# OPPOMKLab/u-LLaVA

Hardware: AMD Instinct MI355X
Metric: images/sec/GPU (ViT-L-336 + LLaMA-7B + SAM RES forward) at 1/2/4/8 MI355X (higher is better)
Workload: dtype bf16; 1 GPU; C4: ViT-L/14-336 + LLaMA-7B instruct forward, 336x336 image + 64-token prompt (S=643), batch 32/GPU; per_gpu_batch=32, global_batch=32, seq_len=643, image=336, parallelism=dp1, weights=random-init N(0,0.02), ViT-L/14 + LLaMA-7B (V=32011) shapes

## Files before the change

### u-llava_amd/csrc/attention.hip

```cpp
#include "ull_common.h"
#include <stdlib.h>
#include <type_traits>

#include "attention_common.h"

namespace {

typedef uint32_t u32x2_t __attribute__((ext_vector_type(2)));
template <int OFF>
ULL_DEV u32x2_t lds_tr_b64(uint32_t addr) {
    u32x2_t v;
    asm volatile("ds_read_b64_tr_b16 %0, %1 offset:%2" : "=v"(v) : "v"(addr), "n"(OFF) : "memory");
    return v;
}
template <int N, int LEFT = 0>
ULL_DEV void lds_tr_wait(u32x2_t (&a)[N], u32x2_t (&b)[N]) {
    static_assert(N == 1 || N == 4 || N == 5 || N == 8, "head-dim blocks of hd = 64 / 80 / 128");
    if constexpr (N == 1)
        asm volatile("s_waitcnt lgkmcnt(%2)" : "+v"(a[0]), "+v"(b[0]) : "n"(LEFT) : "memory");
    else if constexpr (N == 4)
        asm volatile("s_waitcnt lgkmcnt(%8)" : "+v"(a[0]), "+v"(a[1]), "+v"(a[2]), "+v"(a[3]), "+v"(b[0]), "+v"(b[1]), "+v"(b[2]), "+v"(b[3])
                     : "n"(LEFT) : "memory");
    else if constexpr (N == 5)
        asm volatile("s_waitcnt lgkmcnt(%10)"
                     : "+v"(a[0]), "+v"(a[1]), "+v"(a[2]), "+v"(a[3]), "+v"(a[4]), "+v"(b[0]), "+v"(b[1]), "+v"(b[2]), "+v"(b[3]), "+v"(b[4])
                     : "n"(LEFT) : "memory");
    else
        asm volatile("s_waitcnt lgkmcnt(%16)"
                     : "+v"(a[0]), "+v"(a[1]), "+v"(a[2]), "+v"(a[3]), "+v"(a[4]), "+v"(a[5]), "+v"(a[6]), "+v"(a[7]), "+v"(b[0]), "+v"(b[1]),
                       "+v"(b[2]), "+v"(b[3]), "+v"(b[4]), "+v"(b[5]), "+v"(b[6]), "+v"(b[7])
                     : "n"(LEFT) : "memory");
}

template <int HDP, int NT, int NWV, bool EXACT, bool VROW>
constexpr int attn_reg_nbuf() {
    constexpr int ULL_ATTN_RING = 2;
    return EXACT ? 2 * NT : ((VROW && (HDP / 8) % NWV == 0 && NT >= 2) ? ULL_ATTN_RING : 2);
}

template <int HDP, int NT, int FL, int NWV, bool EXACT = false, bool VROW = false>
__global__ __launch_bounds__(NWV * 64, (EXACT || (VROW && HDP == 64 && NWV == 4)) ? 4 : (VROW && HDP == 128 && NT <= 11 && NWV <= 4) ? 3 :
                                       2)
void attn_reg_kernel(AttnArgs p) {
    extern __shared__ __attribute__((aligned(256))) char smem[];
    static_assert(!VROW || ((FL == FL_LLAMA || FL == FL_CLIP) && HDP >= 64), "VROW: flavors that pin hd = HDP");
    constexpr int PM = HDP / 16 >= 8 ? 7 : HDP / 16 - 1;
    constexpr int BQ = 16 * NWV;
    constexpr int CPR = HDP / 8;
    constexpr int KROW = HDP * 2;
    constexpr int NKS = HDP / 32, NDS = HDP / 16;
    constexpr int TILE = 64 * KROW > HDP * 128 ? 64 * KROW : HDP * 128;
    const int tid = threadIdx.x, lane = tid & 63;
    const int hd = head_dim_of<HDP, FL>(p);
    const int wave = __builtin_amdgcn_readfirstlane(tid >> 6);
    const int fr = lane & 15, fg = lane >> 4;

    const int nq = (p.Sq + BQ - 1) / BQ;
    const int xcd = blockIdx.x & 7, slot = blockIdx.x >> 3;
    const int head = (slot / nq) * 8 + xcd;
    if (head >= p.B * p.H) return;
    const int qt = nq - 1 - slot % nq;
    const int b = head / p.H, h = head % p.H;
    const int q0 = qt * BQ;
    const int koff = p.Sk - p.Sq;

    const uint32_t lds_base = __builtin_amdgcn_readfirstlane((uint32_t)(uintptr_t)(__attribute__((address_space(3))) char*)smem);
    constexpr int NBUF = attn_reg_nbuf<HDP, NT, NWV, EXACT, VROW>();
    constexpr int PPW = (CPR + NWV - 1) / NWV;
    char* maskb = smem + NBUF * TILE;
    elem_t* biasb = (elem_t*)(smem + NBUF * TILE + NT * KT);

    int kend = p.Sk;
    if (p.causal) kend = min(p.Sk, q0 + BQ + koff);
    if (kend < 1) kend = 1;
    const int nkt = EXACT ? NT : (kend + KT - 1) / KT;
    int kend_w = p.Sk;
    if (p.causal) kend_w = min(p.Sk, q0 + wave * 16 + 16 + koff);
    int nkt_w = EXACT ? NT : (q0 + wave * 16 < p.Sq) ? max(1, (kend_w + KT - 1) / KT) : 0;

    const elem_t* kbase = p.K + (long)b * p.k_bs + (long)h * p.k_hs;
    const elem_t* vbase = p.Vt + (long)b * p.vt_bs + (long)h * p.vt_hs;
    constexpr bool FASTDMA = VROW && (HDP / 8) % NWV == 0;
    uint32_t kvo[FASTDMA ? 2 * PPW : 1];
    if constexpr (FASTDMA) {
#pragma unroll
        for (int i0 = 0; i0 < PPW; ++i0) {
            const int i = i0 * NWV + wave;
            const int row = i * (64 / CPR) + lane / CPR;
            const int ck = (lane % CPR) ^ swz<CPR>(row);
            const int cpos = lane % CPR;
            const int cv = ((((cpos >> 1) ^ (row & PM)) << 1) | (cpos & 1));
            kvo[i0] = (uint32_t)(((long)row * p.k_ss + ck * 8) * 2);
            kvo[PPW + i0] = (uint32_t)(((long)row * p.vt_ds + cv * 8) * 2);
        }
    }
    const bool fast_dma_ok = FASTDMA && 64 * p.k_ss * 2 < (1L << 31) && 64 * p.vt_ds * 2 < (1L << 31);
    auto issue = [&](int s) {
        const uint32_t dst = lds_base + (EXACT ? s : (s % NBUF)) * TILE;
        if constexpr (FASTDMA) {
            const int kt = s < nkt ? s : s - nkt;
            if (fast_dma_ok && kt * KT + KT <= p.Sk) {
                const elem_t* tb = s < nkt ? kbase + (long)kt * KT * p.k_ss : vbase + (long)kt * KT * p.vt_ds;
#pragma unroll
                for (int i0 = 0; i0 < PPW; ++i0) glds16s(tb, s < nkt ? kvo[i0] : kvo[PPW + i0], dst + (i0 * NWV + wave) * 1024);
                return;
            }
        }
        if (s < nkt) {
            const int kt = s;
#pragma unroll
            for (int i0 = 0; i0 < CPR; i0 += NWV) {
                const int i = i0 + wave;
                if (i < CPR) {
                    const int row = i * (64 / CPR) + lane / CPR;
                    const int c = (lane % CPR) ^ swz<CPR>(row);
                    const int key = min(kt * KT + row, p.Sk - 1);
                    const elem_t* krow = kbase + (long)key * p.k_ss;
                    const elem_t* src = (c * 8 < hd) ? krow + c * 8 : p.zeros;
                    glds16(src, dst + i * 1024);
                }
            }
        } else if constexpr (VROW) {
            const int kt = s - nkt;
#pragma unroll
            for (int i0 = 0; i0 < CPR; i0 += NWV) {
                const int i = i0 + wave;
                if (i < CPR) {
                    const int row = i * (64 / CPR) + lane / CPR;
                    const int cpos = lane % CPR;
                    const int c = ((((cpos >> 1) ^ (row & PM)) << 1) | (cpos & 1));
                    const int key = min(kt * KT + row, p.Sk - 1);
                    glds16(vbase + (long)key * p.vt_ds + c * 8, dst + i * 1024);
                }
            }
        } else {
            const int kt = s - nkt;
            const int npieces = hd >> 3;
#pragma unroll
            for (int i0 = 0; i0 < HDP / 8; i0 += NWV) {
                const int i = i0 + wave;
                if (i < npieces) {
                    const int row = i * 8 + (lane >> 3);
                    const int c = (lane & 7) ^ (row & 7);
                    glds16(vbase + (long)row * p.vt_ds + kt * KT + c * 8, dst + i * 1024);
                }
            }
        }
    };

    if constexpr (EXACT) {
#pragma unroll
        for (int kt = 0; kt < NT; ++kt) issue(kt);
    } else {
#pragma unroll
        for (int s0 = 0; s0 < NBUF - 1; ++s0)
            if (s0 < 2 * nkt) issue(s0);
    }

    uint4 qf[NKS];
    const int qi = q0 + wave * 16 + fr;
    {
        const elem_t* qp = p.Q + (long)b * p.q_bs + (long)h * p.q_hs + (long)qi * p.q_ss;
#pragma unroll
        for (int ks = 0; ks < NKS; ++ks) {
            const int d = ks * 32 + fg * 8;
            qf[ks] = (qi < p.Sq && d < hd) ? *(const uint4*)(qp + d) : make_uint4(0, 0, 0, 0);
        }
        for (int j = tid; j < nkt * KT; j += NWV * 64) {
            unsigned char m = 2;
            if (j < p.Sk) m = (p.key_mask == nullptr || p.key_mask[(long)b * p.Sk + j] != 0) ? 1 : 0;
            maskb[j] = m;
        }
    }
    const elem_t* brow = nullptr;
    int bh_off = 0, bw_off = 0;
    if (p.rel_h != nullptr) {
        const int bp = bias_pitch(p);
        stage_rel_bias<NKS>(p, biasb + wave * 16 * bp, bp, qf, q0 + wave * 16, head, lane, bh_off, bw_off, hd);
        brow = biasb + (wave * 16 + fr) * bp;
    }
    if (p.q_scale != 1.0f) {
#pragma unroll
        for (int ks = 0; ks < NKS; ++ks) qf[ks] = scale_q8(qf[ks], p.q_scale);
    }
    asm volatile("s_waitcnt vmcnt(0)" ::: "memory");
#pragma unroll
    for (int ks = 0; ks < NKS; ++ks) asm volatile("" : "+v"(qf[ks].x), "+v"(qf[ks].y), "+v"(qf[ks].z), "+v"(qf[ks].w));
    float mrow = -INFINITY;
    ULL_ATT_ACC(0, stamp_t);

    uint32_t sp[NT][8];
    uint32_t kfo[NKS];
#pragma unroll
    for (int ks = 0; ks < NKS; ++ks) {
        kfo[ks] = fr * KROW + (((ks * 4 + fg) ^ swz<CPR>(fr)) << 4);
        asm volatile("" : "+v"(kfo[ks]));
    }
    uint32_t vfo = (4 * fg + (fr >> 2)) * KROW + ((fr & 2) << 3) + ((fr & 1) << 3) + (((4 * (fg & 1) + (fr >> 2)) & PM) << 5);
    asm volatile("" : "+v"(vfo));
    if constexpr (EXACT) {
        __builtin_amdgcn_s_barrier();
#pragma unroll
        for (int kt = 0; kt < NT; ++kt) issue(NT + kt);
    }
    auto stream_step = [&](int s) {
        const int total = 2 * nkt;
        const int later = min(NBUF - 2, total - 1 - s);
        if (NBUF >= 4 && later >= 2) asm volatile("s_waitcnt vmcnt(%0)" :: "n"(2 * PPW) : "memory");
        else if (NBUF >= 3 && later == 1) asm volatile("s_waitcnt vmcnt(%0)" :: "n"(PPW) : "memory");
        else asm volatile("s_waitcnt vmcnt(0)" ::: "memory");
        __builtin_amdgcn_s_barrier();
        if (s + NBUF - 1 < total) issue(s + NBUF - 1);
    };

#pragma clang loop unroll(full)
    for (int kt = 0; kt < NT; ++kt) {
        if (kt < nkt) {
            if constexpr (!EXACT) stream_step(kt);
            ULL_ATT_ACC(1, stamp_t);
            if (kt < nkt_w) {
                const char* tb = smem + (EXACT ? kt : (kt % NBUF)) * TILE;
                if constexpr (VROW) {
                    if (p.key_mask == nullptr && kt * KT + KT <= p.Sk && (FL != FL_LLAMA || kt * KT + KT - 1 <= q0 + wave * 16 + koff)) {
constexpr int ULL_ATTN_CHAINS = 2;
#pragma unroll
                        for (int n0 = 0; n0 < 4; n0 += ULL_ATTN_CHAINS) {
                            f32x4_t accn[ULL_ATTN_CHAINS];
#pragma unroll
                            for (int c = 0; c < ULL_ATTN_CHAINS; ++c) accn[c] = f32x4_t{0.f, 0.f, 0.f, 0.f};
#pragma unroll
                            for (int ks = 0; ks < NKS; ++ks)
#pragma unroll
                                for (int c = 0; c < ULL_ATTN_CHAINS; ++c) {
                                    const uint4 kf = *(const uint4*)(tb + (n0 + c) * 16 * KROW + kfo[ks]);
                                    accn[c] = mfma16(kf, qf[ks], accn[c]);
                                }
#pragma unroll
                            for (int c = 0; c < ULL_ATTN_CHAINS; ++c)
                                score_quad_clean<FL>(p, accn[c], sp[kt][(n0 + c) * 2], sp[kt][(n0 + c) * 2 + 1], &mrow);
                        }
                        continue;
                    }
                }
#pragma unroll
                for (int ns = 0; ns < 4; ++ns) {
                    f32x4_t acc = {0.f, 0.f, 0.f, 0.f};
                    const int row = ns * 16 + fr;
#pragma unroll
                    for (int ks = 0; ks < NKS; ++ks) {
                        if (ks * 32 < hd) {
                            const uint4 kf = *(const uint4*)(tb + ns * 16 * KROW + kfo[ks]);
                            acc = mfma16(kf, qf[ks], acc);
                        }
                    }
                    if constexpr (FL == FL_LLAMA || FL == FL_CLIP) {
                        if (p.key_mask == nullptr && kt * KT + KT <= p.Sk && (FL != FL_LLAMA || kt * KT + KT - 1 <= q0 + wave * 16 + koff)) {
                            score_quad_clean<FL>(p, acc, sp[kt][ns * 2], sp[kt][ns * 2 + 1], &mrow);
                            continue;
                        }
                    }
                    const uint32_t mk = *(const uint32_t*)(maskb + kt * KT + ns * 16 + fg * 4);
                    const int j0 = kt * KT + ns * 16 + fg * 4;
                    bool fast = false;
                    if constexpr (FL == FL_LLAMA || FL == FL_CLIP) {
                        const bool dirty = mk != 0x01010101u || (FL == FL_LLAMA && j0 + 3 > qi + koff);
                        fast = __builtin_amdgcn_ballot_w64(dirty) == 0;
                    }
                    if (fast) score_quad_clean<FL>(p, acc, sp[kt][ns * 2], sp[kt][ns * 2 + 1], &mrow);
                    else score_quad<FL>(p, acc, j0, mk, qi, koff, brow, bh_off, bw_off, sp[kt][ns * 2], sp[kt][ns * 2 + 1], &mrow);
                    if constexpr (EXACT) __builtin_amdgcn_sched_barrier(0);
                }
            }
        }
    }

    {
        float m = rnd(mrow);
        m = fmaxf(m, __shfl_xor(m, 16, 64));
        m = fmaxf(m, __shfl_xor(m, 32, 64));
        float sum = 0.f;
#pragma clang loop unroll(full)
        for (int kt = 0; kt < NT; ++kt)
            if (kt < nkt_w) {
#pragma unroll
                for (int i = 0; i < 8; ++i) {
                    const f32x2_t t = (f32x2_t{pk_lo(sp[kt][i]), pk_hi(sp[kt][i])} - m) * 1.4426950408889634f;
                    sum += __builtin_amdgcn_exp2f(t.x);
                    sum += __builtin_amdgcn_exp2f(t.y);
                }
                if constexpr (EXACT) __builtin_amdgcn_sched_barrier(0);
            }
        sum += __shfl_xor(sum, 16, 64);
        sum += __shfl_xor(sum, 32, 64);
        const float inv = 1.0f / sum;
#pragma clang loop unroll(full)
        for (int kt = 0; kt < NT; ++kt)
            if (kt < nkt_w) {
#pragma unroll
                for (int i = 0; i < 8; ++i) {
                    const f32x2_t t = (f32x2_t{pk_lo(sp[kt][i]), pk_hi(sp[kt][i])} - m) * 1.4426950408889634f;
                    const f32x2_t e = f32x2_t{__builtin_amdgcn_exp2f(t.x), __builtin_amdgcn_exp2f(t.y)} * inv;
                    sp[kt][i] = pack2e(e.x, e.y);
                }
                if constexpr (EXACT) __builtin_amdgcn_sched_barrier(0);
            }
    }

    f32x4_t oacc[NDS];
#pragma unroll
    for (int ds = 0; ds < NDS; ++ds) oacc[ds] = f32x4_t{0.f, 0.f, 0.f, 0.f};
    if constexpr (EXACT) {
        asm volatile("s_waitcnt vmcnt(0)" ::: "memory");
        __builtin_amdgcn_s_barrier();
    }
#pragma clang loop unroll(full)
    for (int kt = 0; kt < NT; ++kt) {
        if (kt < nkt) {
            if constexpr (!EXACT) stream_step(nkt + kt);
            ULL_ATT_ACC(4, stamp_t);
            if constexpr (VROW) {
                if (kt < nkt_w) {
                    const uint32_t vb = lds_base + (EXACT ? NT + kt : ((nkt + kt) % NBUF)) * TILE + vfo;
#pragma unroll
                    for (int kk = 0; kk < 2; ++kk) {
                        const uint4 pf = make_uint4(sp[kt][4 * kk], sp[kt][4 * kk + 1], sp[kt][4 * kk + 2], sp[kt][4 * kk + 3]);
#pragma unroll
                        for (int d0 = 0; d0 < NDS; d0 += 4) {
                            u32x2_t va[4], vc[4];
#pragma unroll
                            for (int j = 0; j < 4; ++j) {
                                const uint32_t ad = vb ^ ((d0 + j) << 5);
                                if (kk == 0) { va[j] = lds_tr_b64<0>(ad); vc[j] = lds_tr_b64<16 * KROW>(ad); }
                                else { va[j] = lds_tr_b64<32 * KROW>(ad); vc[j] = lds_tr_b64<48 * KROW>(ad); }
                            }
                            lds_tr_wait<4>(va, vc);
#pragma unroll
                            for (int j = 0; j < 4; ++j)
                                oacc[d0 + j] = mfma16(make_uint4(va[j].x, va[j].y, vc[j].x, vc[j].y), pf, oacc[d0 + j]);
                        }
                    }
                }
            } else
            if (kt < nkt_w) {
                const char* tb = smem + (EXACT ? NT + kt : ((nkt + kt) % NBUF)) * TILE;
#pragma unroll
                for (int kk = 0; kk < 2; ++kk) {
                    const uint4 pf = make_uint4(sp[kt][4 * kk], sp[kt][4 * kk + 1], sp[kt][4 * kk + 2], sp[kt][4 * kk + 3]);
#pragma unroll
                    for (int ds = 0; ds < NDS; ++ds) {
                        if (ds * 16 < hd) {
                            const int row = ds * 16 + fr;
                            const uint4 vf = *(const uint4*)(tb + row * 128 + (((kk * 4 + fg) ^ (row & 7)) << 4));
                            oacc[ds] = mfma16(vf, pf, oacc[ds]);
                        }
                    }
                    if constexpr (EXACT) __builtin_amdgcn_sched_barrier(0);
                }
            }
        }
    }
    if constexpr (VROW && !EXACT && NBUF == 2 && NWV * 16 * KROW <= TILE) {
        char* ob = smem + ((2 * nkt - 2) % NBUF) * TILE + wave * 16 * KROW;
        constexpr int SM = CPR >= 16 ? 15 : CPR - 1;
        int ln = lane;
        asm volatile("" : "+v"(ln));
        const int er = ln & 15, eg = ln >> 4;
#pragma unroll
        for (int ds = 0; ds < NDS; ++ds) {
            uint2 pk;
            pk.x = pack2e(oacc[ds][0], oacc[ds][1]);
            pk.y = pack2e(oacc[ds][2], oacc[ds][3]);
            *(uint2*)(ob + er * KROW + ((((ds * 2 + (eg >> 1)) ^ (er & SM))) << 4) + ((eg & 1) << 3)) = pk;
        }
        constexpr int RPI = 64 / CPR;
        elem_t* ow = p.O + (long)b * p.o_bs + (long)h * p.o_hs;
#pragma unroll
        for (int it = 0; it < 16 / RPI; ++it) {
            const int r = it * RPI + ln / CPR, c = ln % CPR;
            const uint4 v = *(const uint4*)(ob + r * KROW + ((c ^ (r & SM)) << 4));
            const int q = q0 + wave * 16 + r;
            if (q < p.Sq) *(uint4*)(ow + (long)q * p.o_ss + c * 8) = v;
        }
    } else
    if (qi < p.Sq) {
        elem_t* op = p.O + (long)b * p.o_bs + (long)h * p.o_hs + (long)qi * p.o_ss;
#pragma unroll
        for (int ds = 0; ds < NDS; ++ds) {
            if (ds * 16 < hd) {
                uint2 pk;
                pk.x = pack2e(oacc[ds][0], oacc[ds][1]);
                pk.y = pack2e(oacc[ds][2], oacc[ds][3]);
                *(uint2*)(op + ds * 16 + fg * 4) = pk;
            }
        }
    }
}

constexpr int SW_NWV = 13, SW_NT = 4, SW_WS = 14, SW_HD = 80, SW_NTAB = 2 * SW_WS - 1, SW_BW = SW_NTAB + 1, SW_BP = 2 * SW_BW, SW_TILE = 64 * 256;
constexpr int SW_LDS = 2 * SW_NT * SW_TILE + SW_NWV * 16 * SW_BP * 2 + 2 * SW_NTAB * SW_HD * 2;
static_assert(SW_LDS <= 160 * 1024, "K + V tiles, 208 bias rows and the two rel-pos tables fit one CU's LDS");
__global__ __launch_bounds__(SW_NWV * 64) void sam_window_kernel(AttnArgs p, int n_items) {
    extern __shared__ __attribute__((aligned(256))) char smem[];
    constexpr int NWV = SW_NWV, NT = SW_NT, WS = SW_WS, NBLK = SW_WS, KROW = 256, TILE = SW_TILE, NKS = 3, HD = SW_HD, NTAB = SW_NTAB, BW = SW_BW, BP = SW_BP;
    const int tid = threadIdx.x, lane = tid & 63;
    const int wave = __builtin_amdgcn_readfirstlane(tid >> 6);
    const int fr = lane & 15, fg = lane >> 4;
    const uint32_t lds_base = __builtin_amdgcn_readfirstlane((uint32_t)(uintptr_t)(__attribute__((address_space(3))) char*)smem);
    elem_t* biasb = (elem_t*)(smem + 2 * NT * TILE);
    elem_t* tabs = biasb + NWV * 16 * BP;
    elem_t* brow = biasb + (wave * 16 + fr) * BP;

    int item = (int)((uint64_t)blockIdx.x * (uint64_t)n_items / gridDim.x);
    const int last = (int)((uint64_t)(blockIdx.x + 1) * (uint64_t)n_items / gridDim.x);
    if (item >= last) return;

    const int qi = wave * 16 + fr;
    const int qy = min(qi, WS * WS - 1) / WS;
    const elem_t* brow_h = biasb + (wave * 16 + fr) * BP + qy + WS - 1;
    uint32_t kfo[NKS];
#pragma unroll
    for (int ks = 0; ks < NKS; ++ks) {
        kfo[ks] = fr * KROW + (((ks * 4 + fg) ^ (fr & 15)) << 4);
        asm volatile("" : "+v"(kfo[ks]));
    }
    uint32_t vfx = (lds_base + NT * TILE + (4 * fg + (fr >> 2)) * 256 + ((fr & 2) << 3) + ((fr & 1) << 3)) ^ ((4 * (fg & 1) + (fr >> 2)) << 5);
    asm volatile("" : "+v"(vfx));
    const uint32_t row_pitch = (uint32_t)p.img_w * (uint32_t)p.k_ss * 2u;

    struct Item { int h, iy0, ix0; long tok0; };
    auto locate = [&](int it) {
        const int b = udiv_magic(it, p.mg_h);
        const WinOrigin wo = win_origin(p, b, WS);
        return Item{it - b * p.H, wo.iy0, wo.ix0, ((long)wo.img * p.img_h + wo.iy0) * p.img_w + wo.ix0};
    };
    auto issue_tiles = [&](const Item& t, int which) {
        int ln = tid;
        asm volatile("" : "+v"(ln));
        const char* in_base = (const char*)((which ? p.Vt : p.K) + t.tok0 * p.k_ss + (long)t.h * p.k_hs);
        const char* pad_base = (const char*)((which ? p.v_pad : p.k_pad) + (long)t.h * p.k_hs);
#pragma unroll
        for (int j = 0; j < 2; ++j) {
            const int i = wave + j * NWV;
            if (i < 16) {
                const int l4 = (ln >> 4) & 3, cpos = ln & 15, row = i * 4 + l4;
                const uint32_t c = 16u * (uint32_t)(which ? ((((cpos >> 1) ^ (row & 7)) << 1) | (cpos & 1)) : (cpos ^ (row & 15)));
                const int lx = min((i & 3) * 4 + l4, WS - 1);
                const bool real = c < HD * 2;
                const bool col_ok = real && t.ix0 + lx < p.img_w;
                const char* in = in_base + ((uint32_t)lx * (uint32_t)p.k_ss * 2u + c);
                const char* out = real ? pad_base + c : (const char*)p.zeros;
#pragma unroll
                for (int kt = 0; kt < NT; ++kt) {
                    if (kt * 64 + i * 4 >= NBLK * 16) continue;
                    const int ly = kt * 4 + (i >> 2);
                    const bool row_ok = t.iy0 + ly < p.img_h;
                    glds16((row_ok && col_ok) ? in + (uint32_t)ly * row_pitch : out, lds_base + (which * NT + kt) * TILE + i * 1024);
                }
            }
        }
    };
    auto query_pos = [&](const Item& t, int pitch, uint32_t& off, bool& ok) {
        int ln = tid;
        asm volatile("" : "+v"(ln));
        const int q = (ln >> 6) * 16 + (ln & 15), qc = min(q, WS * WS - 1), y = qc / WS, x = qc - y * WS;
        ok = q < WS * WS && t.iy0 + y < p.img_h && t.ix0 + x < p.img_w;
        off = (uint32_t)(y * p.img_w + x) * (uint32_t)pitch * 2u;
    };
    auto load_q = [&](const Item& t, uint4 (&q)[NKS], bool& ok) {
        uint32_t off;
        query_pos(t, (int)p.q_ss, off, ok);
        int ln = tid;
        asm volatile("" : "+v"(ln));
        const int g = (ln >> 4) & 3;
        const char* qb = (const char*)(p.Q + t.tok0 * p.q_ss + (long)t.h * p.q_hs) + (off + g * 16);
#pragma unroll
        for (int ks = 0; ks < NKS; ++ks)
            q[ks] = (ok && ks * 32 + g * 8 < HD) ? *(const uint4*)(qb + ks * 64) : make_uint4(0, 0, 0, 0);
// ... 1319 lines not shown
                sp[t][i] = pack2e(lo, hi);
            }
#pragma unroll
            for (int kk = 0; kk < 2; ++kk) {
                const uint4 pf = make_uint4(sp[t][4 * kk], sp[t][4 * kk + 1], sp[t][4 * kk + 2], sp[t][4 * kk + 3]);
#pragma unroll
                for (int ds = 0; ds < NDS; ++ds) {
                    if (ds * 16 < hd) {
                        uint4 vf;
                        if constexpr (TPW == 1) vf = vpre[kk][ds];
                        else vf = *(const uint4*)(vbase + (long)(ds * 16 + fr) * p.vt_ds + kt * KT + (kk * 4 + fg) * 8);
                        oacc[ds] = mfma16(vf, pf, oacc[ds]);
                    }
                }
            }
        }
    }
#pragma unroll
    for (int ds = 0; ds < NDS; ++ds)
#pragma unroll
        for (int r = 0; r < 4; ++r) obuf[(wave * NDS * 4 + ds * 4 + r) * 64 + lane] = oacc[ds][r];
    __syncthreads();
    for (int e = tid; e < NDS * 4 * 64; e += blockDim.x) {
        float acc = 0.f;
        for (int w = 0; w < nwv; ++w) acc += obuf[w * NDS * 4 * 64 + e];
        const int reg = e >> 6, ln = e & 63;
        const int q = ln & 15, d = (reg >> 2) * 16 + (ln >> 4) * 4 + (reg & 3);
        if (q < p.Sq && d < hd) p.O[(long)b * p.o_bs + (long)h * p.o_hs + (long)q * p.o_ss + d] = f2e(acc);
    }
}

__global__ __launch_bounds__(256) void rope_inplace_kernel(elem_t* __restrict__ x, long row_stride, const int64_t* __restrict__ pos,
                                                           const float* __restrict__ inv_freq, int n_heads, int hd, float sin_sign) {
    const long tok = blockIdx.x;
    const int half = hd >> 1;
    const int cpr = half >> 3;
    const int c = threadIdx.x % cpr;
    const float pf = (float)pos[tok];
    float cs[8], sn[8];
#pragma unroll
    for (int j = 0; j < 8; ++j) {
        const float a = pf * inv_freq[c * 8 + j];
        cs[j] = rnd(cosf(a));
        sn[j] = rnd(sinf(a)) * sin_sign;
    }
    elem_t* xr = x + tok * row_stride;
    for (int hh = threadIdx.x / cpr; hh < n_heads; hh += blockDim.x / cpr) {
        elem_t* p1 = xr + hh * hd + c * 8;
        elem_t* p2 = p1 + half;
        float a[8], bb[8], o1[8], o2[8];
        unpack8(*(const uint4*)p1, a);
        unpack8(*(const uint4*)p2, bb);
#pragma unroll
        for (int j = 0; j < 8; ++j) {
            o1[j] = rnd(a[j] * cs[j]) + rnd(-bb[j] * sn[j]);
            o2[j] = rnd(bb[j] * cs[j]) + rnd(a[j] * sn[j]);
        }
        *(uint4*)p1 = pack8(o1);
        *(uint4*)p2 = pack8(o2);
    }
}

__global__ __launch_bounds__(256) void rope_table_kernel(const int64_t* __restrict__ pos, const float* __restrict__ inv_freq, long tokens,
                                                         int half, elem_t* __restrict__ cs, elem_t* __restrict__ sn) {
    const long total = tokens * half;
    for (long i = (long)blockIdx.x * 256 + threadIdx.x; i < total; i += (long)gridDim.x * 256) {
        const float a = (float)pos[i / half] * inv_freq[i % half];
        cs[i] = f2e(cosf(a));
        sn[i] = f2e(sinf(a));
    }
}

__global__ __launch_bounds__(64) void rope_append_kernel(elem_t* __restrict__ qkv, long row_stride, const int64_t* __restrict__ pos,
                                                         const float* __restrict__ inv_freq, int S, int H, int hd, elem_t* __restrict__ kc,
                                                         elem_t* __restrict__ vtc, int smax, int past) {
    const long tok = blockIdx.x;
    const int h = blockIdx.y;
    const int b = (int)(tok / S), s = (int)(tok % S);
    const int half = hd >> 1;
    const int cpr = half >> 3;
    elem_t* xr = qkv + tok * row_stride;
    const int slot_k = past + s;
    if ((int)threadIdx.x < 2 * cpr) {
        const int c = threadIdx.x % cpr;
        const bool is_k = (int)threadIdx.x >= cpr;
        const float pf = (float)pos[tok];
        float cs[8], sn[8];
#pragma unroll
        for (int j = 0; j < 8; ++j) {
            const float a = pf * inv_freq[c * 8 + j];
            cs[j] = rnd(cosf(a));
            sn[j] = rnd(sinf(a));
        }
        elem_t* p1 = xr + ((is_k ? H : 0) + h) * hd + c * 8;
        elem_t* p2 = p1 + half;
        float a[8], bb[8], o1[8], o2[8];
        unpack8(*(const uint4*)p1, a);
        unpack8(*(const uint4*)p2, bb);
#pragma unroll
        for (int j = 0; j < 8; ++j) {
            o1[j] = rnd(a[j] * cs[j]) + rnd(-bb[j] * sn[j]);
            o2[j] = rnd(bb[j] * cs[j]) + rnd(a[j] * sn[j]);
        }
        const uint4 r1 = pack8(o1), r2 = pack8(o2);
        if (!is_k) {
            *(uint4*)p1 = r1;
            *(uint4*)p2 = r2;
        } else {
            elem_t* kp = kc + (((long)b * H + h) * smax + slot_k) * hd + c * 8;
            *(uint4*)kp = r1;
            *(uint4*)(kp + half) = r2;
        }
    }
    const int w = slot_k & 31;
    const int slot_v = (slot_k & ~31) + 8 * ((w >> 2) & 3) + 4 * (w >> 4) + (w & 3);
    const elem_t* vr = xr + 2 * H * hd + h * hd;
    for (int i = threadIdx.x; i < hd; i += 64) vtc[(((long)b * H + h) * hd + i) * smax + slot_v] = vr[i];
}

__global__ __launch_bounds__(256) void transpose_v_kernel(const elem_t* __restrict__ v, long v_bs, long v_ss, elem_t* __restrict__ vt, int S,
                                                          int H, int hd, int pitch) {
    __shared__ __attribute__((aligned(16))) elem_t t[64][68];
    const int b = blockIdx.z / H, h = blockIdx.z % H;
    const int s0 = blockIdx.x * 64, d0 = blockIdx.y * 64;
    const elem_t* vp = v + (long)b * v_bs + (long)h * hd;
#pragma unroll
    for (int k = 0; k < 2; ++k) {
        const int c = threadIdx.x + 256 * k;
        const int sl = c >> 3, dc = (c & 7) * 8;
        uint4 val = make_uint4(0, 0, 0, 0);
        if (s0 + sl < S && d0 + dc < hd) val = *(const uint4*)(vp + (long)(s0 + sl) * v_ss + d0 + dc);
        const uint32_t w[4] = {val.x, val.y, val.z, val.w};
#pragma unroll
        for (int j = 0; j < 4; ++j) {
            t[dc + 2 * j][sl] = (elem_t)(w[j] & 0xffff);
            t[dc + 2 * j + 1][sl] = (elem_t)(w[j] >> 16);
        }
    }
    __syncthreads();
    elem_t* op = vt + ((long)b * H + h) * hd * pitch;
#pragma unroll
    for (int k = 0; k < 2; ++k) {
        const int c = threadIdx.x + 256 * k;
        const int d = c >> 3, oc = c & 7;
        const int kb = (oc >> 2) * 32 + (oc & 3) * 4;
        const uint2 lo = *(const uint2*)&t[d][kb], hi = *(const uint2*)&t[d][kb + 16];
        if (d0 + d < hd) *(uint4*)(op + (long)(d0 + d) * pitch + s0 + oc * 8) = make_uint4(lo.x, lo.y, hi.x, hi.y);
    }
}

template <int HDP, int NT, int FL, int NWV = 8, bool EXACT = false, bool VROW = false>
int launch_attn(const AttnArgs& a, hipStream_t st) {
    constexpr int TILE = 64 * HDP * 2 > HDP * 128 ? 64 * HDP * 2 : HDP * 128;
    const int lds = attn_reg_nbuf<HDP, NT, NWV, EXACT, VROW>() * TILE + NT * KT +
                    (a.rel_h ? NWV * 16 * (((a.rel_mode == 2 ? 2 * (a.KH + a.KW) - 2 : a.KH + a.KW) | 1)) * 2 + 16 : 0);
    if (lds > 160 * 1024) return ULL_ERR_LDS;
    static UllOncePerDevice once;
    if (lds > 64 * 1024 && once.first())
        (void)hipFuncSetAttribute((const void*)attn_reg_kernel<HDP, NT, FL, NWV, EXACT, VROW>, hipFuncAttributeMaxDynamicSharedMemorySize, 160 * 1024);
    const int nq = (a.Sq + 16 * NWV - 1) / (16 * NWV);
    const int nheads = a.B * a.H;
    const dim3 grid(((nheads + 7) / 8) * 8 * nq);
    hipLaunchKernelGGL((attn_reg_kernel<HDP, NT, FL, NWV, EXACT, VROW>), grid, dim3(NWV * 64), lds, st, a);
    return ull_check_launch();
}

template <int HDP, int FL>
int launch_long(const AttnArgs& a, hipStream_t st) {
    constexpr int TILE = 64 * HDP * 2;
    const int nt = (a.Sk + KT - 1) / KT;
    const int lds = 4 * TILE + ((nt * KT + 15) & ~15) + (a.rel_h ? 8 * 16 * (((a.rel_mode == 2 ? 2 * (a.KH + a.KW) - 2 : a.KH + a.KW) | 1)) * 2 + 16 : 0);
    if (lds > 160 * 1024) return ULL_ERR_LDS;
    static UllOncePerDevice once;
    if (once.first()) (void)hipFuncSetAttribute((const void*)attn_long_kernel<HDP, FL>, hipFuncAttributeMaxDynamicSharedMemorySize, 160 * 1024);
    const int nq = (a.Sq + 127) / 128;
    const dim3 grid(((a.B * a.H + 7) / 8) * 8 * nq);
    hipLaunchKernelGGL((attn_long_kernel<HDP, FL>), grid, dim3(512), lds, st, a);
    return ull_check_launch();
}

template <int HDP, int FL, int HOIST, bool VROW = false>
int launch_stream(const AttnArgs& a, hipStream_t st) {
    constexpr int TILE = 64 * HDP * 2;
    static_assert(!VROW || HOIST == 2, "row-major V: the SAM global-attention form");
    const int nt = (a.Sk + KT - 1) / KT;
    int lds = 4 * TILE;
    if (HOIST == 0) lds += ((nt * KT + 15) & ~15) + (a.rel_h ? 8 * 16 * (((a.rel_mode == 2 ? 2 * (a.KH + a.KW) - 2 : a.KH + a.KW) | 1)) * 2 + 16 : 0);
    if (lds > 160 * 1024) return ULL_ERR_LDS;
    static UllOncePerDevice once;
    if (once.first()) (void)hipFuncSetAttribute((const void*)attn_stream_kernel<HDP, FL, HOIST, VROW>, hipFuncAttributeMaxDynamicSharedMemorySize, 160 * 1024);
    const int nq = (a.Sq + 127) / 128;
    const dim3 grid(((a.B * a.H + 7) / 8) * 8 * nq);
    hipLaunchKernelGGL((attn_stream_kernel<HDP, FL, HOIST, VROW>), grid, dim3(512), lds, st, a);
    return ull_check_launch();
}

int launch_sam_global(const AttnArgs& a, hipStream_t st) {
    constexpr int LDS = 4 * 64 * 256 + 4 * 32 * 64 * 2;
    static UllOncePerDevice once;
    if (once.first()) (void)hipFuncSetAttribute((const void*)sam_global_kernel, hipFuncAttributeMaxDynamicSharedMemorySize, 160 * 1024);
    const int nq = a.Sq / 128;
    const dim3 grid(((a.B * a.H + 7) / 8) * 8 * nq);
    hipLaunchKernelGGL(sam_global_kernel, grid, dim3(256), LDS, st, a);
    return ull_check_launch();
}

int launch_sam_global_exact(const AttnArgs& a, hipStream_t st) {
    constexpr int LDS = 4 * 64 * 256 + 4 * 32 * 64 * 2;
    static UllOncePerDevice once;
    if (once.first()) (void)hipFuncSetAttribute((const void*)sam_global_exact_kernel, hipFuncAttributeMaxDynamicSharedMemorySize, 160 * 1024);
    const int nq = a.Sq / 128;
    const dim3 grid(((a.B * a.H + 7) / 8) * 8 * nq);
    hipLaunchKernelGGL(sam_global_exact_kernel, grid, dim3(256), LDS, st, a);
    return ull_check_launch();
}

template <int HDP, int FL, int TPW>
int launch_fewq_t(const AttnArgs& a, int nwv, hipStream_t st) {
    const int lds = 2 * 16 * 16 * 4 + nwv * HDP * 16 * 4;
    static UllOncePerDevice once;
    if (once.first()) (void)hipFuncSetAttribute((const void*)attn_fewq_kernel<HDP, FL, TPW>, hipFuncAttributeMaxDynamicSharedMemorySize, 160 * 1024);
    hipLaunchKernelGGL((attn_fewq_kernel<HDP, FL, TPW>), dim3(a.B * a.H), dim3(nwv * 64), lds, st, a);
    return ull_check_launch();
}

template <int HDP, int FL>
int launch_fewq(const AttnArgs& a, hipStream_t st) {
    const int nt = (a.Sk + KT - 1) / KT;
    const int nwv = nt < 16 ? nt : 16;
    return nt <= 16 ? launch_fewq_t<HDP, FL, 1>(a, nwv, st) : launch_fewq_t<HDP, FL, 4>(a, nwv, st);
}

int flavor_of(const AttnArgs& a) {
    if (a.scale_mode == 1 && a.causal && !a.rel_h && a.q_scale == 1.0f) return FL_LLAMA;
    if (a.scale_mode == 1 && !a.causal && !a.rel_h && !a.key_mask && a.q_scale == 1.0f) return FL_CLIP;
    if (a.scale_mode == 0 && !a.causal && a.rel_h && !a.key_mask) return FL_SAM_ENC;
    if (a.scale_mode == 2 && !a.causal && !a.rel_h && !a.key_mask && a.q_scale == 1.0f) return FL_SAM_DEC;
    return FL_RUNTIME;
}

template <int HDP>
int dispatch_nt(const AttnArgs& a, hipStream_t st) {
    const int nt = (a.Sk + KT - 1) / KT;
    int fl = flavor_of(a);
    if ((fl == FL_LLAMA || fl == FL_CLIP) && a.hd != HDP) fl = FL_RUNTIME;
    if (fl == FL_SAM_ENC && HDP == 128 && a.hd != 80) fl = FL_RUNTIME;
    if (a.v_rows) {
        if constexpr (HDP == 128) {
            constexpr int ULL_ATTN_NWV = 4;
            if (fl == FL_LLAMA && a.Sq > 16 && nt <= 11) return launch_attn<128, 11, FL_LLAMA, ULL_ATTN_NWV, false, true>(a, st);
            if (fl == FL_LLAMA && a.Sq > 16 && nt <= 16) return launch_attn<128, 16, FL_LLAMA, 8, false, true>(a, st);
            if (fl == FL_SAM_ENC && a.rel_mode == 2 && a.KW == 64 && a.KH == 64 && a.Sk == 4096 && (a.Sq & 15) == 0 && a.Sq > 16 &&
                64 * a.k_ss * 2 < (1L << 31) && 64 * a.vt_ds * 2 < (1L << 31)) {
                if ((a.Sq & 127) == 0 && a.Sq == a.Sk && a.hd == 80 && !a.key_mask && !a.causal) return launch_sam_global(a, st);
                return launch_stream<128, FL_SAM_ENC, 2, true>(a, st);
            }
        }
        if constexpr (HDP == 64) {
            if (fl == FL_CLIP && a.Sq > 16 && nt <= 5) return launch_attn<64, 5, FL_CLIP, 8, false, true>(a, st);
            if (fl == FL_CLIP && a.Sq > 16 && nt <= 11) return launch_attn<64, 11, FL_CLIP, 4, false, true>(a, st);
        }
        return ULL_ERR_SHAPE;
    }
    if (a.Sq <= 16 && !a.rel_h && nt >= 2 && nt <= 64) {
        if constexpr (HDP == 128) {
            if (fl == FL_LLAMA) return launch_fewq<HDP, FL_LLAMA>(a, st);
        }
        if constexpr (HDP == 32) {
            if (fl == FL_SAM_DEC) return launch_fewq<HDP, FL_SAM_DEC>(a, st);
        }
        return launch_fewq<HDP, FL_RUNTIME>(a, st);
    }
    if constexpr (HDP == 128) {
        if (fl == FL_LLAMA && nt <= 11) return launch_attn<128, 11, FL_LLAMA, 4>(a, st);
        if (fl == FL_LLAMA && nt <= 16) return launch_attn<128, 16, FL_LLAMA>(a, st);
        if (a.win16) {
            if (fl != FL_SAM_ENC || a.KH != 14 || a.KW != 14 || a.Sk != 196 || a.Sq != 196 || a.key_mask) return ULL_ERR_SHAPE;
            const int n_items = a.B * a.H, n_cu = ull_cu_count();
            static UllOncePerDevice once;
            if (once.first()) (void)hipFuncSetAttribute((const void*)sam_window_kernel, hipFuncAttributeMaxDynamicSharedMemorySize, 160 * 1024);
            hipLaunchKernelGGL(sam_window_kernel, dim3(n_items < n_cu ? n_items : n_cu), dim3(SW_NWV * 64), SW_LDS, st, a, n_items);
            return ull_check_launch();
        }
        if (fl == FL_SAM_ENC && nt == 4 && a.Sq <= 208) return launch_attn<128, 4, FL_SAM_ENC, 13, true>(a, st);
        if (fl == FL_SAM_ENC && nt <= 11) return launch_attn<128, 11, FL_SAM_ENC>(a, st);
        if (fl == FL_SAM_ENC && nt > 16) {
            if (a.rel_mode == 1 && a.KW == KT && (a.Sk % KT) == 0) return launch_stream<128, FL_SAM_ENC, 1>(a, st);
            if (a.rel_mode == 2 && a.KW == 64 && a.KH == 64 && a.Sk == 4096 && (a.Sq & 15) == 0) return launch_stream<128, FL_SAM_ENC, 2>(a, st);
            return launch_stream<128, FL_SAM_ENC, 0>(a, st);
        }
    }
    if constexpr (HDP == 64) {
        if (fl == FL_CLIP && nt <= 5) return launch_attn<64, 5, FL_CLIP>(a, st);
        if (fl == FL_CLIP && nt <= 11) return launch_attn<64, 11, FL_CLIP, 4>(a, st);
    }
    if constexpr (HDP == 32) {
        if (fl == FL_SAM_DEC && nt <= 5) return launch_attn<32, 5, FL_SAM_DEC>(a, st);
        if (fl == FL_SAM_DEC && nt > 16) return launch_long<32, FL_SAM_DEC>(a, st);
    }
    if constexpr (HDP < 128) {
        if (nt <= 5) return launch_attn<HDP, 5, FL_RUNTIME>(a, st);
    }
    if (nt <= 11) return launch_attn<HDP, 11, FL_RUNTIME>(a, st);
    if (nt <= 16) return launch_attn<HDP, 16, FL_RUNTIME>(a, st);
    return launch_long<HDP, FL_RUNTIME>(a, st);
}

// ... 143 lines not shown
```

Before: 143.6 images/sec (whole job, all GPUs).

## Skip masked causal key groups and detect all-ones key masks in attention

Each block now checks at load time whether the key mask holds any zeros, and shares that flag through LDS so an all-ones mask can take the unmasked fast score path. For causal and CLIP variants, it also skips the QK MFMAs, the exp work and half of the PV MFMAs for 16-key groups that lie entirely past the wave's causal limit. Those groups get constant fill scores. The skip is only used when the row max is far enough above the fill value that skipped entries would contribute nothing. The cost is extra branches, a ballot and a barrier-dependent LDS read, plus 16 more bytes of LDS.

```diff
diff --git a/u-llava_amd/csrc/attention.hip b/u-llava_amd/csrc/attention.hip
--- a/u-llava_amd/csrc/attention.hip
+++ b/u-llava_amd/csrc/attention.hip
@@ -77,6 +77,11 @@
     int kend_w = p.Sk;
     if (p.causal) kend_w = min(p.Sk, q0 + wave * 16 + 16 + koff);
     int nkt_w = EXACT ? NT : (q0 + wave * 16 < p.Sq) ? max(1, (kend_w + KT - 1) / KT) : 0;
+    constexpr bool GROUPS = VROW && !EXACT && (FL == FL_LLAMA || FL == FL_CLIP);
+    const int ng_w = nkt_w > 0 ? max(1, (kend_w + 15) >> 4) : 0;
+    constexpr bool MFLAG = FL == FL_LLAMA && !EXACT;
+    char* cleanb = smem + NBUF * TILE + NT * KT;
+    bool mclean = p.key_mask == nullptr;
 
     const elem_t* kbase = p.K + (long)b * p.k_bs + (long)h * p.k_hs;
     const elem_t* vbase = p.Vt + (long)b * p.vt_bs + (long)h * p.vt_hs;
@@ -166,10 +171,28 @@
             const int d = ks * 32 + fg * 8;
             qf[ks] = (qi < p.Sq && d < hd) ? *(const uint4*)(qp + d) : make_uint4(0, 0, 0, 0);
         }
-        for (int j = tid; j < nkt * KT; j += NWV * 64) {
-            unsigned char m = 2;
-            if (j < p.Sk) m = (p.key_mask == nullptr || p.key_mask[(long)b * p.Sk + j] != 0) ? 1 : 0;
-            maskb[j] = m;
+        constexpr int MI = (NT * KT + NWV * 64 - 1) / (NWV * 64);
+        int mw[MI];
+#pragma unroll
+        for (int it = 0; it < MI; ++it) {
+            const int j = tid + it * NWV * 64;
+            mw[it] = (p.key_mask != nullptr && j < nkt * KT && j < p.Sk) ? p.key_mask[(long)b * p.Sk + j] : 1;
+        }
+        bool mzero = false;
+#pragma unroll
+        for (int it = 0; it < MI; ++it) {
+            const int j = tid + it * NWV * 64;
+            if (j < nkt * KT) {
+                const unsigned char m = j < p.Sk ? (mw[it] != 0 ? 1 : 0) : 2;
+                maskb[j] = m;
+                mzero |= m == 0;
+            }
+        }
+        if constexpr (MFLAG) {
+            if (p.key_mask != nullptr) {
+                const bool wclean = __builtin_amdgcn_ballot_w64(mzero) == 0;
+                if (lane == 0) cleanb[wave] = wclean ? 1 : 0;
+            }
         }
     }
     const elem_t* brow = nullptr;
@@ -218,10 +241,18 @@
         if (kt < nkt) {
             if constexpr (!EXACT) stream_step(kt);
             ULL_ATT_ACC(1, stamp_t);
+            if constexpr (MFLAG) {
+                if (kt == 0 && p.key_mask != nullptr) {
+                    bool c = true;
+#pragma unroll
+                    for (int w = 0; w < NWV; ++w) c &= cleanb[w] != 0;
+                    mclean = __builtin_amdgcn_readfirstlane(c) != 0;
+                }
+            }
             if (kt < nkt_w) {
                 const char* tb = smem + (EXACT ? kt : (kt % NBUF)) * TILE;
                 if constexpr (VROW) {
-                    if (p.key_mask == nullptr && kt * KT + KT <= p.Sk && (FL != FL_LLAMA || kt * KT + KT - 1 <= q0 + wave * 16 + koff)) {
+                    if (mclean && kt * KT + KT <= p.Sk && (FL != FL_LLAMA || kt * KT + KT - 1 <= q0 + wave * 16 + koff)) {
 constexpr int ULL_ATTN_CHAINS = 2;
 #pragma unroll
                         for (int n0 = 0; n0 < 4; n0 += ULL_ATTN_CHAINS) {
@@ -244,6 +275,18 @@
                 }
 #pragma unroll
                 for (int ns = 0; ns < 4; ++ns) {
+                    if constexpr (GROUPS) {
+                        if (kt * 4 + ns >= ng_w) {
+                            const int j0 = kt * KT + ns * 16 + fg * 4;
+                            float o[4];
+#pragma unroll
+                            for (int r = 0; r < 4; ++r) o[r] = j0 + r < p.Sk ? ELEM_MIN_F : -INFINITY;
+                            mrow = fmaxf(mrow, o[0]);
+                            sp[kt][ns * 2] = pack2e(o[0], o[1]);
+                            sp[kt][ns * 2 + 1] = pack2e(o[2], o[3]);
+                            continue;
+                        }
+                    }
                     f32x4_t acc = {0.f, 0.f, 0.f, 0.f};
                     const int row = ns * 16 + fr;
 #pragma unroll
@@ -254,7 +297,7 @@
                         }
                     }
                     if constexpr (FL == FL_LLAMA || FL == FL_CLIP) {
-                        if (p.key_mask == nullptr && kt * KT + KT <= p.Sk && (FL != FL_LLAMA || kt * KT + KT - 1 <= q0 + wave * 16 + koff)) {
+                        if (mclean && kt * KT + KT <= p.Sk && (FL != FL_LLAMA || kt * KT + KT - 1 <= q0 + wave * 16 + koff)) {
                             score_quad_clean<FL>(p, acc, sp[kt][ns * 2], sp[kt][ns * 2 + 1], &mrow);
                             continue;
                         }
@@ -274,19 +317,35 @@
         }
     }
 
+    int ng_phase3 = 0;
     {
         float m = rnd(mrow);
         m = fmaxf(m, __shfl_xor(m, 16, 64));
         m = fmaxf(m, __shfl_xor(m, 32, 64));
+        int ng_p = ng_w;
+        if constexpr (GROUPS) {
+            const bool far = m - ELEM_MIN_F > 256.0f && m < INFINITY;
+            if (__builtin_amdgcn_ballot_w64(!far) != 0) ng_p = nkt_w * 4;
+        }
         float sum = 0.f;
 #pragma clang loop unroll(full)
         for (int kt = 0; kt < NT; ++kt)
             if (kt < nkt_w) {
-#pragma unroll
-                for (int i = 0; i < 8; ++i) {
-                    const f32x2_t t = (f32x2_t{pk_lo(sp[kt][i]), pk_hi(sp[kt][i])} - m) * 1.4426950408889634f;
-                    sum += __builtin_amdgcn_exp2f(t.x);
-                    sum += __builtin_amdgcn_exp2f(t.y);
+                if (!GROUPS || kt * 4 + 4 <= ng_p) {
+#pragma unroll
+                    for (int i = 0; i < 8; ++i) {
+                        const f32x2_t t = (f32x2_t{pk_lo(sp[kt][i]), pk_hi(sp[kt][i])} - m) * 1.4426950408889634f;
+                        sum += __builtin_amdgcn_exp2f(t.x);
+                        sum += __builtin_amdgcn_exp2f(t.y);
+                    }
+                } else {
+#pragma unroll
+                    for (int i = 0; i < 8; ++i)
+                        if (kt * 4 + i / 2 < ng_p) {
+                            const f32x2_t t = (f32x2_t{pk_lo(sp[kt][i]), pk_hi(sp[kt][i])} - m) * 1.4426950408889634f;
+                            sum += __builtin_amdgcn_exp2f(t.x);
+                            sum += __builtin_amdgcn_exp2f(t.y);
+                        }
                 }
                 if constexpr (EXACT) __builtin_amdgcn_sched_barrier(0);
             }
@@ -296,14 +355,28 @@
 #pragma clang loop unroll(full)
         for (int kt = 0; kt < NT; ++kt)
             if (kt < nkt_w) {
-#pragma unroll
-                for (int i = 0; i < 8; ++i) {
-                    const f32x2_t t = (f32x2_t{pk_lo(sp[kt][i]), pk_hi(sp[kt][i])} - m) * 1.4426950408889634f;
-                    const f32x2_t e = f32x2_t{__builtin_amdgcn_exp2f(t.x), __builtin_amdgcn_exp2f(t.y)} * inv;
-                    sp[kt][i] = pack2e(e.x, e.y);
+                if (!GROUPS || kt * 4 + 4 <= ng_p) {
+#pragma unroll
+                    for (int i = 0; i < 8; ++i) {
+                        const f32x2_t t = (f32x2_t{pk_lo(sp[kt][i]), pk_hi(sp[kt][i])} - m) * 1.4426950408889634f;
+                        const f32x2_t e = f32x2_t{__builtin_amdgcn_exp2f(t.x), __builtin_amdgcn_exp2f(t.y)} * inv;
+                        sp[kt][i] = pack2e(e.x, e.y);
+                    }
+                } else {
+#pragma unroll
+                    for (int i = 0; i < 8; ++i) {
+                        if (kt * 4 + i / 2 < ng_p) {
+                            const f32x2_t t = (f32x2_t{pk_lo(sp[kt][i]), pk_hi(sp[kt][i])} - m) * 1.4426950408889634f;
+                            const f32x2_t e = f32x2_t{__builtin_amdgcn_exp2f(t.x), __builtin_amdgcn_exp2f(t.y)} * inv;
+                            sp[kt][i] = pack2e(e.x, e.y);
+                        } else {
+                            sp[kt][i] = 0;
+                        }
+                    }
                 }
                 if constexpr (EXACT) __builtin_amdgcn_sched_barrier(0);
             }
+        if constexpr (GROUPS) ng_phase3 = ng_p;
     }
 
     f32x4_t oacc[NDS];
@@ -323,6 +396,9 @@
                     const uint32_t vb = lds_base + (EXACT ? NT + kt : ((nkt + kt) % NBUF)) * TILE + vfo;
 #pragma unroll
                     for (int kk = 0; kk < 2; ++kk) {
+                        if constexpr (GROUPS) {
+                            if (kk == 1 && kt * 4 + 2 >= ng_phase3) continue;
+                        }
                         const uint4 pf = make_uint4(sp[kt][4 * kk], sp[kt][4 * kk + 1], sp[kt][4 * kk + 2], sp[kt][4 * kk + 3]);
 #pragma unroll
                         for (int d0 = 0; d0 < NDS; d0 += 4) {
@@ -1948,7 +2024,7 @@
 template <int HDP, int NT, int FL, int NWV = 8, bool EXACT = false, bool VROW = false>
 int launch_attn(const AttnArgs& a, hipStream_t st) {
     constexpr int TILE = 64 * HDP * 2 > HDP * 128 ? 64 * HDP * 2 : HDP * 128;
-    const int lds = attn_reg_nbuf<HDP, NT, NWV, EXACT, VROW>() * TILE + NT * KT +
+    const int lds = attn_reg_nbuf<HDP, NT, NWV, EXACT, VROW>() * TILE + NT * KT + (FL == FL_LLAMA ? 16 : 0) +
                     (a.rel_h ? NWV * 16 * (((a.rel_mode == 2 ? 2 * (a.KH + a.KW) - 2 : a.KH + a.KW) | 1)) * 2 + 16 : 0);
     if (lds > 160 * 1024) return ULL_ERR_LDS;
     static UllOncePerDevice once;
```

New measurement: 143.8 images/sec (whole job, all GPUs) (median of 6 runs). Within noise of the previous version (+0.1%).
